# zz9tf/multimodal-fusion

Measured on AMD Instinct MI355X. Metric: similarity-pairs/sec (NxN cosine+top-k), higher is better.
Workload: dtype f16 MFMA scan + f32 exact re-rank; 1 GPU; N=262144 d=512 single-modality cosine + top-5, self excluded, f32 features, unit-norm Gaussian rows; rows_per_rank=262144, parallelism=single GPU, driver=single, scan_kernel=scan_b16x<f16> (v_mfma_f32_16x16x32_f16), col_splits=1, scan_grid=2048, fallback_rows=0, overflow_rows=0, query_order=False, near_duplicate_rows_estimate=0

## Files before the change

multimodal-fusion_amd/csrc/mmf_api.hip:

```cpp
#include <stdarg.h>
#include <string.h>

#include <algorithm>
#include <map>
#include <mutex>
#include <optional>
#include <utility>
#include <vector>

#include "mmf_host.h"

namespace mmf {

static thread_local char g_err[512] = "";

void set_error(const char* fmt, ...) {
  va_list ap;
  va_start(ap, fmt);
  vsnprintf(g_err, sizeof(g_err), fmt, ap);
  va_end(ap);
}

struct WsEntry { char* base = nullptr; size_t cap = 0; WsKept kept; };
static std::mutex g_ws_mu;
// ... 213 lines not shown

static void fill_stats(mmf_simtopk_stats* st, int precision, int splits, int grid, float prep_ms, float scan_ms, float rerank_ms,
                       float fallback_ms, int64_t fallback_rows, int64_t overflow_rows, int64_t short_rows,
                       const std::vector<uint32_t>& h_tot, int64_t near_rows = -1) {
  if (!st) return;
  st->precision_used = precision; st->col_splits = splits; st->scan_grid = grid;
  st->prep_ms = prep_ms; st->scan_ms = scan_ms; st->rerank_ms = rerank_ms; st->fallback_ms = fallback_ms;
  st->fallback_rows = fallback_rows; st->overflow_rows = overflow_rows; st->short_rows = short_rows;
  for (uint32_t v : h_tot) st->candidates += v;
  st->near_rows = near_rows;
}

static constexpr int kSpillCap = 192;

static size_t b16_lists_bytes(int64_t n, int lists, int bcap) {
  const size_t e = (size_t)n * lists;
  return ws_bytes(e, 4) + ws_bytes(e * bcap, 4) + (lists > 2 ? ws_bytes(e * bcap, 4) + ws_bytes(n, 4) : 0) + 2 * ws_bytes(n, 4) +
         ws_bytes((size_t)n * kSpillCap, 4);
}
static CandLists carve_b16_lists(Workspace& ws, int64_t n, int lists, int bcap) {
  CandLists L{};
  L.lists = lists; L.cap = bcap; L.slot_ulp = scan_bf16_slot_ulp(bcap); L.spill_cap = kSpillCap;
  L.cnt = ws.take<uint32_t>((size_t)n * lists); L.ids = ws.take<uint32_t>((size_t)n * lists * bcap);
  if (lists > 2) { L.keys = ws.take<float>((size_t)n * lists * bcap); L.margin = ws.take<float>(n); }
  L.overflow = ws.take<uint32_t>(n); L.spill_cnt = ws.take<uint32_t>(n); L.spill_ids = ws.take<uint32_t>((size_t)n * kSpillCap);
  L.spill_stacks = (lists == 2 && !getenv("MMF_SPILL_COUNTER")) ? 1 : 0;
  return L;
}

struct FlagBlock {
  int32_t* fail_rows = nullptr; uint32_t *fail_count = nullptr, *cand_total = nullptr;
  uint32_t h_fail4[4] = {0, 0, 0, 0};
  std::vector<uint32_t> h_tot;
  static size_t bytes(int64_t n) { return ws_bytes(n, 4) + ws_bytes(4, 4) + ws_bytes(256, 4); }
  void carve(Workspace& ws, int64_t n) { fail_rows = ws.take<int32_t>(n); fail_count = ws.take<uint32_t>(4); cand_total = ws.take<uint32_t>(256); }
  int zero(hipStream_t s) const {
    MMF_HIP(hipMemsetAsync(fail_count, 0, 16, s)); MMF_HIP(hipMemsetAsync(cand_total, 0, 1024, s));
    return MMF_OK;
  }
  int read(bool totals, hipStream_t s) {
    MMF_HIP(hipMemcpyAsync(h_fail4, fail_count, 16, hipMemcpyDeviceToHost, s));
    h_tot.assign(totals ? 256 : 0, 0);
    if (totals) MMF_HIP(hipMemcpyAsync(h_tot.data(), cand_total, 1024, hipMemcpyDeviceToHost, s));
    MMF_HIP(hipStreamSynchronize(s));
    return MMF_OK;
  }
};

static void symmetric_live_mode(bool* live, bool* forward) {
  const char* e = getenv("MMF_SYMMETRIC_LIVE");
  const int v = e ? atoi(e) : 1;
  *live = (v == 1 || v == 2);
  *forward = (v == 0 || v == 2);
}
static constexpr int64_t kSymMinRows = 131072;
static bool symmetric_scan_wanted(int64_t n, int dp, int bcap, int metric, int forced_splits, bool same_ids, int* G) {
  if (!same_ids || dp != 512 || bcap != scan_bf16_cap(1, 512) || forced_splits != 0) return false;
  if (metric != MMF_DOT && metric != MMF_COSINE) return false;
  const int64_t nb = (n + 255) / 256;
  if (nb * 256 * 1024 >= (int64_t(1) << 32)) return false;
  const char* e = getenv("MMF_SYMMETRIC");
  const int mode = e ? atoi(e) : -1;
  if (mode == 0 || (mode < 0 && n < kSymMinRows)) return false;
  int g = sym_default_group(nb);
  if (const char* ge = getenv("MMF_SYMMETRIC_G")) { const int v = atoi(ge); if (v >= 1 && v <= 65536) g = v; }
  *G = g;
  return true;
}


struct ExactLists {
  CandLists L{};
  int32_t* fail_rows = nullptr; uint32_t* fail_count = nullptr;
  float* floor_key = nullptr; uint32_t* floor_id = nullptr;
  int64_t rows = 0;
  static size_t bytes(int64_t rows, size_t list_words, int cap, bool floors) {
    return ws_bytes(list_words, 4) + ws_bytes(list_words * cap, 4) + (floors ? 4 : 2) * ws_bytes(rows, 4) + ws_bytes(4, 4);
  }
  void carve(Workspace& ws, int64_t rows_, size_t list_words, int cap, bool floors) {
    rows = rows_;
    L.cnt = ws.take<uint32_t>(list_words); L.ids = ws.take<uint32_t>(list_words * cap); L.overflow = ws.take<uint32_t>(rows);
    fail_rows = ws.take<int32_t>(rows); fail_count = ws.take<uint32_t>(4);
    if (floors) { floor_key = ws.take<float>(rows); floor_id = ws.take<uint32_t>(rows); }
  }
  int zero(hipStream_t s) const {
    MMF_HIP(hipMemsetAsync(fail_count, 0, 16, s)); MMF_HIP(hipMemsetAsync(L.overflow, 0, (size_t)rows * 4, s));
    return MMF_OK;
  }
};

struct ExactGroup {
  int64_t row0, rows;
  bool gathered;
  int64_t col0, cols;
  int k;
};

struct ExactPass {
  static constexpr int64_t kBatch = 4096;
  const Request& r;
  const float *rx, *cy;
  bool same = false;
  int forced_splits = 0;
  const int32_t* row_ids = nullptr;
  int64_t n_ids = 0;
  uint32_t* cand_total = nullptr;
// ... 192 lines not shown
  void carve(Workspace& ws) {
    L = carve_b16_lists(ws, n, lists_alloc, bcap);
    if (sym_try) {
      sym_cnt = ws.take<uint32_t>(n); sym_ids = ws.take<uint32_t>((size_t)n * kSymCap); sym_keys = ws.take<float>((size_t)n * kSymCap);
      sym.carve(ws, n_pad_q(), sym_grid());
      sym_kept = ws.kept; sym_keep = ws.keep;
    }
    flags.carve(ws, n);
    XL.carve(ws, FB, (size_t)FB * 2 * fb_splits, cap, false);
    scan_scratch = ws.take<char>(scan_scratch_bytes());
    seed = ws.take<int32_t>(2 * n_seed);
    row_keys = ws.take<float>((size_t)rows_exact_cap * m);
    order_scratch = ws.take<char>(select_order_bytes(n));
    if (order_try) {
      qo_scratch = ws.take<char>(query_order_bytes(n));
      qo_Z = ws.take<uint16_t>((size_t)n_pad_q() * dp);
      qo_zn = ws.take<float>(n_pad_q()); qo_rn = ws.take<float>(n_pad_q()); qo_un = ws.take<float>(n_pad_q());
    }
  }
  int run(const Request& r, const FastOperands& fo_in, void* select_wait_event) {
    const hipStream_t s = r.call.s;
    const bool profile = r.profile;
    FastOperands fo = fo_in;
    query_order_forget();
    EventTimer t_order;
    int64_t near_rows = -1;
    if (order_try) {
      MMF_TRY(t_order.start(profile, s));
      MMF_TRY(launch_query_order_probe(fo.ZQ, fo.q_zn, n, fo.dp, fo.f16, qo_scratch, &near_rows, s));
      if (order_mode == MMF_QUERY_ORDER_ON || near_rows >= 8 * (int64_t)query_order_pivots()) {
        MMF_TRY(launch_query_order_apply(fo.ZQ, fo.q_zn, fo.q_rn, fo.q_un, n, n_pad_q(), fo.dp, fo.f16, qo_scratch, qo_Z, qo_zn, qo_rn, qo_un, &fo.perm, s));
        fo.ZQ = qo_Z; fo.q_zn = qo_zn; fo.q_rn = qo_rn; fo.q_un = qo_un;
      }
      MMF_TRY(t_order.stop(s));
    }
    const bool symmetric = sym_try && !fo.perm && fo.n_panels == 0;
    const CandLists L = view(symmetric);
    MMF_HIP(hipMemsetAsync(L.overflow, 0, (size_t)n * 4, s));
    MMF_TRY(flags.zero(s));
    EventTimer t_scan, t_sel, t_fb;
    EventTimer t_panel[16];
    int grid = 0;
    MMF_HIP(hipMemsetAsync(seed, 0x80, (size_t)n_seed * 8, s));
    MMF_HIP(hipMemsetAsync(L.spill_cnt, 0, (size_t)n * 4, s));
    MMF_TRY(t_scan.start(profile, s));
    ScanB16Panel pn;
    pn.seed = seed; pn.seed_stride = n_seed;
    pn.share = (splits > 1 || fo.n_panels > 1) ? 1 : 0;
    if (symmetric) {
      bool live, forward;
      symmetric_live_mode(&live, &forward);
      const WsKept tables{sym.sched, (n + 255) / 256, sym_G, forward ? 1 : 0};
      MMF_TRY(launch_scan_b16_sym(fo.ZC, fo.c_cb, fo.q_zn, fo.q_rn, fo.q_un, fo.max_c, n, r.d, fo.f16, r.metric, kk, sym_G, live, forward,
                                  !(sym_kept == tables), L, scan_scratch, sym, pn, s, &grid));
      if (sym_keep) *sym_keep = tables;
    } else if (fo.n_panels == 0) {
      MMF_TRY(launch_scan_b16(fo.ZQ, fo.ZC, fo.c_cb, fo.q_zn, fo.q_rn, fo.q_un, fo.max_c, n, m, fo.m_pad_tiles, fo.dp, r.d, fo.f16,
                              r.metric, kk, splits, L, scan_scratch, pn, s, &grid));
    } else {
      int list_base = 0;
      for (int p = 0; p < fo.n_panels; ++p) {
        const mmf_panel& P = fo.panels[p];
        if (P.ready_event) MMF_HIP(hipStreamWaitEvent(s, static_cast<hipEvent_t>(P.ready_event), 0));
        MMF_TRY(t_panel[p].start(profile, s));
        pn.list_base = list_base;
        list_base += 2 * panel_splits[p];
        pn.seg_len = (uint32_t)P.seg_len; pn.seg_stride = (uint32_t)P.seg_stride; pn.id_off = (uint32_t)P.id_base;
        MMF_TRY(launch_scan_b16(fo.ZQ, P.Z, P.cb, fo.q_zn, fo.q_rn, fo.q_un, fo.max_c, n, P.m, P.m_pad, fo.dp, r.d, fo.f16,
                                r.metric, kk, panel_splits[p], L, scan_scratch, pn, s, &grid));
        MMF_TRY(t_panel[p].stop(s));
      }
    }
    MMF_TRY(launch_scan_b16_audit(pn, L.overflow, n, s));
    if (const char* e = getenv("MMF_DEBUG_FLAG_ROWS")) {
      const int64_t f = atoll(e);
      if (f > 0) MMF_HIP(hipMemsetAsync(L.overflow, 1, (size_t)(f < n ? f : n) * 4, s));
    }
    MMF_TRY(t_scan.stop(s));
    if (symmetric && getenv("MMF_SYMMETRIC_DEBUG")) {
      MMF_HIP(hipStreamSynchronize(s));
      std::vector<uint32_t> hc((size_t)n), hl((size_t)sym_grid() * 8);
      uint32_t none = 0;
      MMF_HIP(hipMemcpy(hc.data(), sym_cnt, hc.size() * 4, hipMemcpyDeviceToHost));
      MMF_HIP(hipMemcpy(hl.data(), sym.log_cnt, hl.size() * 4, hipMemcpyDeviceToHost));
      MMF_HIP(hipMemcpy(&none, sym.none_cnt, 4, hipMemcpyDeviceToHost));
      unsigned long long tot = 0; uint32_t mx = 0, lmx = 0;
      for (uint32_t v : hc) { tot += v; if (v > mx) mx = v; }
      for (uint32_t v : hl) if (v > lmx) lmx = v;
      bool live, forward;
      symmetric_live_mode(&live, &forward);
      fprintf(stderr, "[mmf symmetric] G %d grid %lld %s %s: rows without a threshold %u, received entries %llu (%.1f per row, largest %u of %d), fullest wave log %u of %d\n",
              sym_G, (long long)sym_grid(), live ? "live" : "frozen", forward ? "ahead" : "back", none, tot, (double)tot / (double)n, mx,
              kSymCap, lmx, kSymLogPerWave);
    }
    if (select_wait_event) MMF_HIP(hipStreamWaitEvent(s, static_cast<hipEvent_t>(select_wait_event), 0));

    SelectProblem q = r.select();
    q.rx = fo.rx; q.cy = fo.cy; q.perm = fo.perm;
    q.fail_rows = flags.fail_rows; q.fail_count = flags.fail_count; q.cand_total = r.stats ? flags.cand_total : nullptr;
    q.two_pass = true;
    q.order_scratch = getenv("MMF_SELECT_UNORDERED") ? nullptr : order_scratch;
    MMF_TRY(t_sel.start(profile, s));
    MMF_TRY(launch_select(q, L, s));
    MMF_TRY(t_sel.stop(s));

    MMF_TRY(flags.read(r.stats != nullptr, s));
    const uint32_t* h_fail4 = flags.h_fail4;
    const uint32_t h_fail = h_fail4[0];
    if (h_fail > 0 && getenv("MMF_DEBUG_PRINT_FLAGGED")) {
      const uint32_t nshow = h_fail < 8 ? h_fail : 8;
      int32_t rows[8];
      MMF_HIP(hipMemcpy(rows, flags.fail_rows, nshow * sizeof(int32_t), hipMemcpyDeviceToHost));
      for (uint32_t i = 0; i < nshow; ++i) {
        int32_t enc[2] = {0, 0};
        MMF_HIP(hipMemcpy(&enc[0], seed + rows[i], 4, hipMemcpyDeviceToHost));
        MMF_HIP(hipMemcpy(&enc[1], seed + n_seed + rows[i], 4, hipMemcpyDeviceToHost));
        auto dec = [](int32_t o) { int32_t b = o >= 0 ? o : (o ^ 0x7fffffff); float f; memcpy(&f, &b, 4); return f; };
        fprintf(stderr, "[mmf flagged] row %d: best threshold %.9g (enc %d)  best dropped key %.9g (enc %d)  overflow %u short %u\n",
                rows[i], dec(enc[0]), enc[0], dec(enc[1]), enc[1], h_fail4[1], h_fail4[2]);
      }
    }

    MMF_TRY(t_fb.start(profile && h_fail > 0, s));
    if (h_fail > 0 && (int64_t)h_fail <= kRowsExactMax) {
      for (int64_t off = 0; off < (int64_t)h_fail; off += rows_exact_cap) {
        SelectProblem fq = q;
        fq.perm = nullptr;
        fq.row_ids = flags.fail_rows + off;
        fq.n_rows = ((int64_t)h_fail - off < rows_exact_cap) ? ((int64_t)h_fail - off) : rows_exact_cap;
        MMF_TRY(launch_rows_exact(fq, row_keys, s));
      }
    } else if (h_fail > 0) {
      ExactPass ex(r, fo.rx, fo.cy);
      ex.row_ids = flags.fail_rows; ex.n_ids = h_fail; ex.forced_splits = fb_splits;
      ex.add(ExactGroup{0, (int64_t)h_fail, true, 0, m, r.k});
      Workspace aux;
      MMF_TRY(r.call.workspace(ex.image_bytes(), &aux, 1));
      MMF_TRY(XL.zero(s));
      MMF_TRY(ex.run(aux, XL));
    }
    MMF_TRY(t_fb.stop(s));
    fill_stats(r.stats, r.precision, symmetric ? 1 : splits, grid, 0.f, t_scan.ms(), t_sel.ms(), t_fb.ms(), h_fail, h_fail4[1], h_fail4[2], flags.h_tot,
               near_rows);
    if (r.stats) {
      if (profile && fo.n_panels > 0) {
        float launches = 0.f;
// ... 1086 lines not shown
```

multimodal-fusion_amd/csrc/mmf_host.h:

```cpp
#pragma once
#include <hip/hip_runtime.h>
#include <functional>
#include <optional>
#include <stdint.h>
#include <stdio.h>

#include <string>
#include <vector>

#include "../../include/mmf_hg.h"

namespace mmf {

void set_error(const char* fmt, ...);

#define MMF_HIP(call)                                                                      \
  do {                                                                                     \
    hipError_t _e = (call);                                                                \
    if (_e != hipSuccess) {                                                                \
      mmf::set_error("%s failed: %s (%s:%d)", #call, hipGetErrorString(_e), __FILE__, __LINE__); \
      return MMF_E_HIP;                                                                    \
    }                                                                                      \
  } while (0)

// ... 162 lines not shown
  int col_splits;
  const float* floor_key = nullptr;
  const uint32_t* floor_id = nullptr;
};

int scan_f32_cap(int kk);
int launch_scan_f32(const ScanProblem& p, const CandLists& L, hipStream_t s, int* grid_out);

struct SelectProblem {
  const void* X; int64_t n; const void* Y; int64_t m; int64_t d; int dtype; int metric; float lambda;
  int k; int exclude_self; int64_t row_offset; int64_t col_offset;
  const float* rx; const float* cy;
  const int32_t* row_ids; int64_t n_rows;
  int64_t* out_idx; float* out_val;
  int32_t* fail_rows; uint32_t* fail_count;
  uint32_t* cand_total;
  bool two_pass = false;
  int out_stride = 0, out_off = 0;
  float* floor_key_out = nullptr;
  uint32_t* floor_id_out = nullptr;
  void* order_scratch = nullptr;
  const int32_t* perm = nullptr;
};
size_t select_order_bytes(int64_t n);
size_t query_order_bytes(int64_t n);
int query_order_pivots();
int query_order_last(int32_t* out_host, int64_t n);
void query_order_forget();
int launch_query_order_probe(const uint16_t* ZQ, const float* q_zn, int64_t n, int dp, bool f16, void* scratch, int64_t* near, hipStream_t s);
int launch_query_order_apply(const uint16_t* ZQ, const float* q_zn, const float* q_rn, const float* q_un, int64_t n, int64_t n_pad,
                             int dp, bool f16, void* scratch, uint16_t* Zo, float* zno, float* rno, float* uno, const int32_t** perm,
                             hipStream_t s);
int launch_select(const SelectProblem& p, const CandLists& L, hipStream_t s);
int launch_rows_exact(const SelectProblem& p, float* keys, hipStream_t s);
int launch_topk_merge(const int64_t* ia, const float* va, const int64_t* ib, const float* vb,
                      int64_t n, int k, int64_t* io, float* vo, hipStream_t s);
int launch_edge_cosine_impl(const void* X, int64_t d, int dtype, const float* nrm, const int64_t* ei, int64_t E,
                            float* out, hipStream_t s);

int scan_bf16_supported(int64_t d, int kk, int dtype);
int scan_bf16_cap(int kk, int dp);
int scan_bf16_dp(int64_t d);
int launch_prep_half(const void* X, int64_t n, int64_t d, int dtype, int metric, const float* scal,
                     const uint32_t* max_n, void* Z,
                     int64_t n_pad, int dp, int z_f16, float* zn, float* rn, float* un, float* cb, uint32_t* maxima,
                     hipStream_t s);
int launch_scan_b16(const void* ZQ, const void* ZC, const float* cb, const float* q_zn, const float* q_rn,
                    const float* q_un, const uint32_t* maxima, int64_t n_rows, int64_t m, int64_t m_pad, int dp,
                    int64_t d, bool f16, int metric, int kk, int col_splits, const CandLists& L, void* scratch,
                    const ScanB16Panel& pn, hipStream_t s, int* grid_out);
int launch_scan_b16_audit(const ScanB16Panel& pn, uint32_t* overflow, int64_t n_rows, hipStream_t s);
size_t scan_b16_sym_scratch_bytes(int64_t n_rows, int G);
int launch_scan_b16_sym(const void* ZC, const float* cb, const float* zn, const float* rn, const float* un, const uint32_t* maxima,
                        int64_t n, int64_t d, bool f16, int metric, int kk, int G, bool live, bool forward, bool tables,
                        const CandLists& L, void* scratch, const SymBuffers& sb, const ScanB16Panel& pn, hipStream_t s, int* grid_out);
size_t scan_b16_scratch_bytes(int64_t n_rows, int col_splits, int dp, int cap);
int scan_bf16_slot_ulp(int cap);
int scan_b16_queries_per_block(int dp);
int launch_prep_half_gather(const void* X, int64_t n, int64_t d, int dtype, int metric, const float* scal,
                            const uint32_t* max_n, const int32_t* gather, void* Z, int64_t n_pos, int64_t n_pad, int dp,
                            int z_f16, float* zn, float* rn, float* un, float* cb, uint32_t* maxima, hipStream_t s);
size_t scan_b16_seg_scratch_bytes(int64_t grid, int dp, int cap);
int launch_scan_b16_seg(const void* ZQ, const void* ZC, const float* cb, const float* q_zn, const float* q_rn,
                        const float* q_un, const uint32_t* maxima, const int32_t* sched, int64_t grid, int64_t n_rows,
                        int64_t m, int dp, int64_t d, bool f16, int metric, int kk, const CandLists& L, void* scratch,
                        const ScanB16Panel& pn, hipStream_t s);

bool sim_dense_needs_images(int64_t d, int metric);
int launch_sim_dense(const void* X, int64_t n, const void* Y, int64_t m, int64_t d, int dtype,
                     int metric, float lambda, const float* rx, const float* cy, const float* Xp, const float* Yp,
                     float* out, hipStream_t s);
int launch_sim_dense_combined(const float* Fp, const float* P, int64_t n, int64_t d, int64_t dp,
                              float lambda_h, float lambda_g, const float* nf, int64_t row0, int64_t rows, float* out,
                              hipStream_t s);
std::vector<int64_t> sim_dense_combined_seg_table(const int64_t* ptr, int64_t S);
int launch_sim_dense_combined_seg(const float* Fp, const float* P, int64_t d, int64_t dp, float lambda_h, float lambda_g,
                                  const float* nf, const int64_t* sched, int64_t grid, float* out, hipStream_t s);

using MedianConsume = std::function<int(const float* data, int64_t cols, int64_t row0, int64_t rows)>;
using MedianSweep = std::function<int(const MedianConsume&)>;
using MedianSampler = std::function<int(float* sample, int s)>;
size_t median_scratch_bytes(unsigned long long count);
int64_t median_no_diagonal_row();
struct SweepCarry {
  void* lanes;
  int64_t grid;
  int64_t row0;
};
int lower_median_of(unsigned long long count, const MedianSampler& sampler, const MedianSweep& sweep, float* out, void* scratch,
                    hipStream_t s, void* stat_part = nullptr, const float* stat_pivot = nullptr, int64_t* stat_nparts = nullptr,
                    SweepCarry* carry = nullptr);
bool median_one_sweep(unsigned long long count);
size_t stat_lanes_bytes(int64_t grid);
int launch_stat_lanes_init(void* lanes, int64_t grid, hipStream_t s);
int launch_stat_lanes_finish(void* lanes, int64_t grid, void* part , hipStream_t s);
int64_t stats_partial_grid(int64_t count);
int launch_stats_partial_carry(const float* v, int64_t count, int64_t group0, const float* pivot, void* lanes, int64_t grid, hipStream_t s);
int launch_sample_gather(const float* data, int64_t n_sq, unsigned long long count, float* sample, int s_count, hipStream_t s);
int launch_sample_pairs(const void* A, const void* B, int64_t nb, int64_t d, int dtype, float lambda, const float* P, int dp,
                        float lambda_g, int offdiag, unsigned long long count, float* sample, int s_count, hipStream_t s);
int launch_offdiag_lower_median(const float* K, int64_t n, float* out, void* scratch ,
                                hipStream_t s);
int launch_median_accumulate(const float* K, int64_t n, int64_t row0, int64_t rows, void* state, int pass, hipStream_t s);
int launch_median_next(void* state, int pass, float* out, hipStream_t s);
int launch_median_begin_count(void* state, unsigned long long count, hipStream_t s);
int launch_lower_median(const float* v, int64_t count, float* out, void* scratch, hipStream_t s);
int launch_stats_finish(const void* part, int64_t nparts, const float* pivot, int64_t count, double* out, hipStream_t s);
// ... 71 lines not shown
```

multimodal-fusion_amd/csrc/mmf_scan_bf16.hip:

```cpp
#include <stdlib.h>

#include <type_traits>

#include "mmf_dev.h"
#include "mmf_host.h"

namespace mmf {

constexpr int B_CT = 32;
#ifndef MMF_B_CAP
#define MMF_B_CAP 15
#endif
constexpr int B_CAP = MMF_B_CAP;
constexpr int B_CAP_BIG = 16;
constexpr int B_CAP_WIDE = 32;

typedef __bf16 bf16x8_t __attribute__((ext_vector_type(8)));
typedef _Float16 f16x8_t __attribute__((ext_vector_type(8)));
typedef uint32_t u32x4 __attribute__((ext_vector_type(4)));

struct PrepArgs {
  const void* X; int64_t n; int64_t d; int dtype; int metric;
  const float* scal;
  const uint32_t* max_n;
// ... 111 lines not shown
  const void* ZC;
  const float* cb;
  const float* q_zn; const float* q_rn; const float* q_un;
  const uint32_t* maxima;
  int64_t n_rows;
  int64_t m;
  int64_t tiles_total;
  int64_t tiles_per_split;
  int64_t row_blocks;
  int col_splits;
  int conc_splits;
  int64_t blocks_per_round;
  int lists_total;
  int list_base;
  uint32_t seg_len, seg_stride, id_off;
  int32_t* seed;
  int32_t* lost;
  int share;
  int kk;
  int metric;
  int d;
  int debug;
  unsigned long long* dbg;
  uint32_t* lids;
  uint32_t* cand_cnt; uint32_t* cand_ids; uint32_t* overflow;
  float* cand_keys;
  float* margin_out;
  uint32_t* spill_cnt; uint32_t* spill_ids; int spill_cap;
  int spill_stacks;
  const int32_t* sched;
  float* sym_thr;
  int sym_live;
  uint32_t* sym_log;
  uint32_t* sym_log_cnt;
  int sym_log_cap;
};

enum { SEG_QPOS = 0, SEG_ROW0 = 1, SEG_NQ = 2, SEG_T0 = 3, SEG_T1 = 4, SEG_IDOFF = 5, SEG_ENTRY = 8 };
enum { SYM_RB = 0, SYM_B1 = 1, SYM_N1 = 2, SYM_B2 = 3, SYM_N2 = 4 };

__device__ __forceinline__ int32_t seed_enc(float f) {
  const int32_t b = __float_as_int(f);
  return b >= 0 ? b : (b ^ 0x7fffffff);
}
constexpr int32_t kSeedNone = (int32_t)0x80808080;

__device__ __forceinline__ void glds4(const void* gptr, const void* lptr) {
  __builtin_amdgcn_global_load_lds((const __attribute__((address_space(1))) void*)(gptr), (__attribute__((address_space(3))) void*)(lptr), 4, 0, 0);
}

#ifndef MMF_SYM_ABLATE
#define MMF_SYM_ABLATE 0
#endif
template <int KS, bool F16, bool DBG, int NW, int TPB, int CAP, bool SPLITK = false, bool SEG = false, int SYM = 0>
__global__ __launch_bounds__(64 * NW, (NW == 8) ? 2 : 1) void scan_b16x_kernel(ScanB16Args a) {
  static_assert(!SPLITK || (TPB == 1 && NW == 8 && (KS % 8) == 0), "split-k pairs");
  static_assert(SYM == 0 || (!SPLITK && !SEG && !DBG && TPB == 2), "symmetric schedule: the d = 512 kernel only");
  constexpr int NQW = SPLITK ? NW / 2 : NW;
  constexpr int NTL = 64 * NQW;
  constexpr int QT = 32 * NQW;
  constexpr int STAGES = 2 * TPB;
  constexpr int ROWB = KS * 32;
  constexpr int TILEB = B_CT * ROWB;
  constexpr int PIECES = TILEB / 1024;
  constexpr int PPW = (PIECES + NW - 1) / NW;
  static_assert(PIECES % NW == 0, "piece distribution");
  extern __shared__ __attribute__((aligned(1024))) char smem[];
  char* tiles = smem;
  float* cbs = reinterpret_cast<float*>(smem + STAGES * TILEB);
  float* lkeys = cbs + STAGES * 64;
  uint32_t* lids = a.lids + (size_t)blockIdx.x * (SlotList<CAP, NTL>::SLOTS * NTL);
  f32x4* xch = reinterpret_cast<f32x4*>(lkeys + CAP * NTL);
  volatile int* ack = reinterpret_cast<volatile int*>(xch + NQW * 4 * 64);

  const int tid = threadIdx.x;
  const int lane = tid & 63;
  const int wave = __builtin_amdgcn_readfirstlane(tid >> 6);
  const int khalf = SPLITK ? wave / NQW : 0;
  const int qw = SPLITK ? wave % NQW : wave;
  const bool owner = khalf == 0;
  const int half = lane >> 5;
  const int g = lane >> 4;
  const int c16 = lane & 15;
  const int ownb = g & 1;
  const int c = c16 + 16 * ownb;

  int64_t rb;
  int split;
  int64_t t_begin, t_end, row0 = 0;
  int nq = 0;
  uint32_t id_off = a.id_off;
  int sym_n1 = 0, sym_skip = 0;
  if constexpr (SYM != 0) {
    const int32_t* e = a.sched + (size_t)blockIdx.x * SEG_ENTRY;
    if (e[SYM_RB] < 0) return;
    rb = e[SYM_RB]; split = 0;
    t_begin = e[SYM_B1]; t_end = t_begin + e[SYM_N1] + e[SYM_N2];
    sym_n1 = e[SYM_N1]; sym_skip = e[SYM_B2] - (e[SYM_B1] + e[SYM_N1]);
  } else if constexpr (SEG) {
    const int32_t* e = a.sched + (size_t)blockIdx.x * SEG_ENTRY;
    rb = e[SEG_QPOS] / QT; row0 = e[SEG_ROW0]; nq = e[SEG_NQ];
    t_begin = e[SEG_T0]; t_end = e[SEG_T1]; id_off = (uint32_t)e[SEG_IDOFF];
    split = 0;
  } else {
    const int CS = a.conc_splits;
    const int64_t round = blockIdx.x / a.blocks_per_round;
// ... 67 lines not shown
  u32x4 qf[KS2][2];
  {
    const char* qbase = reinterpret_cast<const char*>(a.ZQ) + (q0 + 32 * qw + c16) * (int64_t)ROWB + g * 16 + kbyte;
#pragma unroll
    for (int s = 0; s < KS2; ++s) {
      qf[s][0] = *reinterpret_cast<const u32x4*>(qbase + s * 64);
      qf[s][1] = *reinterpret_cast<const u32x4*>(qbase + 16 * (int64_t)ROWB + s * 64);
    }
#pragma unroll
    for (int s = 0; s < KS2; ++s) { asm volatile("" : "+v"(qf[s][0])); asm volatile("" : "+v"(qf[s][1])); }
  }

  int lo[4];
#pragma unroll
  for (int j = 0; j < 4; ++j) lo[j] = c16 * ROWB + ((((4 * j + g) ^ c16) & 15) << 4);

  uint32_t src_off[PPW];
#pragma unroll
  for (int i = 0; i < PPW; ++i) {
    const int p = wave + NW * i;
    const int off = p * 1024 + lane * 16;
    const int r = off / ROWB;
    const int chunk = (off % ROWB) >> 4;
    const int src_chunk = (chunk & ~15) | ((chunk ^ r) & 15);
    src_off[i] = (uint32_t)(r * ROWB + src_chunk * 16);
  }
  const char* zc0 = reinterpret_cast<const char*>(a.ZC) + (SYM != 0 ? 0 : t_begin * (int64_t)TILEB);
  const char* cb0 = reinterpret_cast<const char*>(a.cb + (SYM != 0 ? 0 : t_begin * B_CT));
  const char* zt0 = SYM != 0 ? zc0 + t_begin * (int64_t)TILEB : zc0;
  const char* ct0 = SYM != 0 ? cb0 + t_begin * B_CT * 4 : cb0;
  const __amdgpu_buffer_rsrc_t zrsrc = __builtin_amdgcn_make_buffer_rsrc(const_cast<char*>(zc0), 0, -1, 0x00020000);
  auto issue_piece = [&](const char* tsrc, int stage, int i) {
    if (DBG && (a.debug & 2)) return;
    if (DBG && (a.debug & 32)) tsrc = zc0;
    __builtin_amdgcn_raw_ptr_buffer_load_lds(zrsrc, (__attribute__((address_space(3))) void*)(tiles + stage * TILEB + (wave + NW * i) * 1024),
                                             16, (int)src_off[i], (int)(uint32_t)(tsrc - zc0), 0, 0);
  };
  const __amdgpu_buffer_rsrc_t brsrc = __builtin_amdgcn_make_buffer_rsrc(const_cast<char*>(cb0), 0, -1, 0x00020000);
  auto issue_bias = [&](const char* bsrc, int stage) {
    const uint32_t l = __builtin_amdgcn_mbcnt_hi(~0u, __builtin_amdgcn_mbcnt_lo(~0u, 0u));
    if (l < 32)
      __builtin_amdgcn_raw_ptr_buffer_load_lds(brsrc, (__attribute__((address_space(3))) void*)(cbs + stage * 64), 4, (int)(l * 4u),
                                               (int)(uint32_t)(bsrc - cb0), 0, 0);
  };
  auto sym_thr_stage = [&](int stage) -> float* { return lkeys + CAP * NTL + stage * 32; };
  auto issue_thr = [&](const char* bsrc, int stage) {
    const __amdgpu_buffer_rsrc_t trsrc = __builtin_amdgcn_make_buffer_rsrc(a.sym_thr, 0, -1, 0x00020000);
    const uint32_t l = __builtin_amdgcn_mbcnt_hi(~0u, __builtin_amdgcn_mbcnt_lo(~0u, 0u));
    if (l < 32)
      __builtin_amdgcn_raw_ptr_buffer_load_lds(trsrc, (__attribute__((address_space(3))) void*)sym_thr_stage(stage), 4, (int)(l * 4u),
                                               (int)(uint32_t)(bsrc - cb0), 0, 16);
  };

  if (SPLITK && tid < NQW) ack[tid] = -1;
  const int Ti = (int)T;
  if (Ti > 0) {
#pragma unroll
    for (int u = 0; u < TPB; ++u) {
      const bool real = u < Ti;
#pragma unroll
      for (int i = 0; i < PPW; ++i) issue_piece(real ? zt0 + u * (int64_t)TILEB : zc0, u, i);
      if (wave == (u & (NW - 1))) issue_bias(real ? ct0 + u * B_CT * 4 : cb0, u);
      if constexpr (SYM == 2) { if (wave == ((u + 4) & (NW - 1))) issue_thr(real ? ct0 + u * B_CT * 4 : cb0, u); }
    }
  }
  constexpr int GRP = KS2 / PPW;
  static_assert(KS2 % PPW == 0 && GRP >= 1, "DMA piece placement");
  const char* tsrc = zt0 + TPB * (int64_t)TILEB;
  const char* bsrc = ct0 + TPB * B_CT * 4;
  const uint32_t id_base = (uint32_t)(t_begin * B_CT);

  struct Acc { f32x4 t[2][2]; };
  auto tile_body = [&](const char* tb, const float* cbt, const char* src, int s2) -> Acc {
    Acc acc;
#pragma unroll
    for (int cb = 0; cb < 2; ++cb) {
      f32x4 b4 = *reinterpret_cast<const f32x4*>(cbt + 16 * cb + 4 * g);
      if (SPLITK && !owner) b4 = f32x4{0.f, 0.f, 0.f, 0.f};
      acc.t[cb][0] = b4; acc.t[cb][1] = b4;
    }
    constexpr int PD = 2;
    u32x4 af[PD][2];
#pragma unroll
    for (int s = 0; s < PD; ++s) {
      af[s][0] = *reinterpret_cast<const u32x4*>(tb + lo[s & 3] + (s >> 2) * 256);
      af[s][1] = *reinterpret_cast<const u32x4*>(tb + lo[s & 3] + (s >> 2) * 256 + 16 * ROWB);
    }
    __builtin_amdgcn_sched_group_barrier(0x100, 2 * PD, 0);
#pragma unroll
    for (int s = 0; s < KS2; ++s) {
      const u32x4 a0 = af[s % PD][0], a1 = af[s % PD][1];
      if (s + PD < KS2) {
        af[s % PD][0] = *reinterpret_cast<const u32x4*>(tb + lo[(s + PD) & 3] + ((s + PD) >> 2) * 256);
        af[s % PD][1] = *reinterpret_cast<const u32x4*>(tb + lo[(s + PD) & 3] + ((s + PD) >> 2) * 256 + 16 * ROWB);
      }
      if constexpr (F16) {
        acc.t[0][0] = __builtin_amdgcn_mfma_f32_16x16x32_f16(__builtin_bit_cast(f16x8_t, a0), __builtin_bit_cast(f16x8_t, qf[s][0]), acc.t[0][0], 0, 0, 0);
        acc.t[0][1] = __builtin_amdgcn_mfma_f32_16x16x32_f16(__builtin_bit_cast(f16x8_t, a0), __builtin_bit_cast(f16x8_t, qf[s][1]), acc.t[0][1], 0, 0, 0);
        acc.t[1][0] = __builtin_amdgcn_mfma_f32_16x16x32_f16(__builtin_bit_cast(f16x8_t, a1), __builtin_bit_cast(f16x8_t, qf[s][0]), acc.t[1][0], 0, 0, 0);
        acc.t[1][1] = __builtin_amdgcn_mfma_f32_16x16x32_f16(__builtin_bit_cast(f16x8_t, a1), __builtin_bit_cast(f16x8_t, qf[s][1]), acc.t[1][1], 0, 0, 0);
      } else {
        acc.t[0][0] = __builtin_amdgcn_mfma_f32_16x16x32_bf16(__builtin_bit_cast(bf16x8_t, a0), __builtin_bit_cast(bf16x8_t, qf[s][0]), acc.t[0][0], 0, 0, 0);
        acc.t[0][1] = __builtin_amdgcn_mfma_f32_16x16x32_bf16(__builtin_bit_cast(bf16x8_t, a0), __builtin_bit_cast(bf16x8_t, qf[s][1]), acc.t[0][1], 0, 0, 0);
        acc.t[1][0] = __builtin_amdgcn_mfma_f32_16x16x32_bf16(__builtin_bit_cast(bf16x8_t, a1), __builtin_bit_cast(bf16x8_t, qf[s][0]), acc.t[1][0], 0, 0, 0);
        acc.t[1][1] = __builtin_amdgcn_mfma_f32_16x16x32_bf16(__builtin_bit_cast(bf16x8_t, a1), __builtin_bit_cast(bf16x8_t, qf[s][1]), acc.t[1][1], 0, 0, 0);
      }
      if ((s % GRP) == GRP - 1) issue_piece(src, s2, s / GRP);
      if (s + PD < KS2) __builtin_amdgcn_sched_group_barrier(0x100, 2, 0);
      __builtin_amdgcn_sched_group_barrier(0x008, 4, 0);
    }
    return acc;
  };
  auto max_qb = [&](const Acc& x, int qb) -> float {
    const f32x4& p = x.t[0][qb];
    const f32x4& q = x.t[1][qb];
    return fmaxf(fmaxf(fmaxf(p[0], p[1]), fmaxf(p[2], p[3])), fmaxf(fmaxf(q[0], q[1]), fmaxf(q[2], q[3])));
  };
  float thr_q0, thr_q1;
  auto refresh_thr = [&]() {
    const float mine = list.thr;
    const float theirs = __shfl_xor(mine, 16);
    thr_q0 = ownb ? theirs : mine;
    thr_q1 = ownb ? mine : theirs;
  };
  refresh_thr();

  auto filter = [&](const Acc& acc, int tt, float m0, float m1) {
    if (__builtin_expect(!(DBG && (a.debug & 1)) && __any((m0 >= thr_q0) || (m1 >= thr_q1)), 0)) {
      uint32_t id0 = id_base + (uint32_t)tt * B_CT;
      if constexpr (SYM != 0) id0 += (tt >= sym_n1) ? (uint32_t)(sym_skip * B_CT) : 0u;
      f32x16 v;
#pragma unroll
      for (int cb = 0; cb < 2; ++cb) {
#pragma unroll
        for (int j = 0; j < 4; ++j) {
          const float mine = ownb ? acc.t[cb][1][j] : acc.t[cb][0][j];
          const float give = ownb ? acc.t[cb][0][j] : acc.t[cb][1][j];
          v[4 * cb + j] = mine;
          v[8 + 4 * cb + j] = __shfl_xor(give, 16);
        }
      }
      const int g4 = 4 * g;
      auto rowof = [g4](int r) -> uint32_t { return (uint32_t)((g4 ^ ((r & 8) >> 1)) + (r & 3) + 16 * ((r >> 2) & 1)); };
      const bool cold = (!seeded && tt < 32) || __any(list.thr == -kFltMax);
      if (DBG && (a.debug & 8)) {
        const bool willc = __any(list.cnt >= CAP - 1);
        int nh = 0;
#pragma unroll
        for (int r = 0; r < 16; ++r) nh += (v[r] >= list.thr) ? 1 : 0;
        const int lanes_hit = __popcll(__ballot(nh > 0));
#pragma unroll
        for (int o = 32; o > 0; o >>= 1) nh += __shfl_xor(nh, o);
        if (lane == 0) {
          atomicAdd(a.dbg + 0, 1ull);
          atomicAdd(a.dbg + 1, cold ? 1ull : 0ull);
          atomicAdd(a.dbg + 2, (unsigned long long)nh);
          atomicAdd(a.dbg + 3, (!cold && willc) ? 1ull : 0ull);
          atomicAdd(a.dbg + 4, (unsigned long long)lanes_hit);
        }
      }
      unsigned long long ts0 = 0;
      if (DBG && (a.debug & 16)) ts0 = __builtin_amdgcn_s_memtime();
      list.offer_tile(v, id0, rowof, a.kk, margin);
      if (DBG && (a.debug & 16) && lane == 0) {
        const unsigned long long dt = __builtin_amdgcn_s_memtime() - ts0;
        atomicAdd(a.dbg + (cold ? 4 : 5), dt);
        atomicAdd(a.dbg + (cold ? 6 : 7), 1ull);
      }
      refresh_thr();
// ... 53 lines not shown
        }
        sym_wcnt += (uint32_t)__popcll(busy);
        busy = __ballot(m != 0u);
      }
    }
  };

  unsigned long long tw = 0, tf = 0, tc = 0, tv = 0, t0s = 0, t1s = 0, t2s = 0, t3s = 0, tvs = 0;
  const bool stamps = DBG && (a.debug & 16) != 0;
  Acc acc_prev;
  float m0_prev = kNegInf, m1_prev = kNegInf;
#pragma unroll
  for (int cb = 0; cb < 2; ++cb) {
#pragma unroll
    for (int j = 0; j < 4; ++j) { acc_prev.t[cb][0][j] = kNegInf; acc_prev.t[cb][1][j] = kNegInf; }
  }
  const int nIter = (Ti + TPB - 1) / TPB;
  for (int j = 0; j < nIter; ++j) {
    if (stamps) tvs = __builtin_amdgcn_s_memtime();
    __builtin_amdgcn_s_waitcnt(0x0F70);
    if (stamps) t0s = __builtin_amdgcn_s_memtime();
    asm volatile("" ::: "memory");
    if (!(DBG && (a.debug & 4)))
    __builtin_amdgcn_s_barrier();
    asm volatile("" ::: "memory");
    if (stamps) t1s = __builtin_amdgcn_s_memtime();

    if constexpr (SPLITK) {
      if (owner) {
        if (j > 0) {
#pragma unroll
          for (int i = 0; i < 4; ++i) {
            const f32x4 p = xch[(qw * 4 + i) * 64 + lane];
            acc_prev.t[i >> 1][i & 1] += p;
          }
          m0_prev = max_qb(acc_prev, 0);
          m1_prev = max_qb(acc_prev, 1);
        }
        asm volatile("" ::: "memory");
        if (lane == 0) ack[qw] = j;
      }
    }
    if (owner) filter(acc_prev, j * TPB - 1, m0_prev, m1_prev);
    if (stamps) t2s = __builtin_amdgcn_s_memtime();

    const int sg = (j & 1) * TPB, ng = TPB - sg;
#pragma unroll
    for (int u = 0; u < TPB; ++u) {
      const int t = j * TPB + u;
      const bool more = (t + TPB < Ti);
      const char* src = more ? tsrc + u * (int64_t)TILEB : zc0;
      Acc acc;
      acc = tile_body(tiles + (sg + u) * TILEB + kbyte, cbs + (sg + u) * 64, src, ng + u);
      if (wave == ((t + TPB) & (NW - 1))) issue_bias(more ? bsrc + u * B_CT * 4 : cb0, ng + u);
      if constexpr (SYM == 2 && MMF_SYM_ABLATE != 2) {
        if (wave == ((t + TPB + 4) & (NW - 1))) issue_thr(more ? bsrc + u * B_CT * 4 : cb0, ng + u);
        if (t < Ti) sym_offer(acc, t, sym_thr_stage(sg + u));
      }
      if (u < TPB - 1) {
        if (TPB == 2 || __builtin_expect(t < Ti, 1))
        filter(acc, t, max_qb(acc, 0), max_qb(acc, 1));
      } else {
        if (__builtin_expect(t >= Ti, 0)) {
#pragma unroll
          for (int cb = 0; cb < 2; ++cb) {
#pragma unroll
            for (int jj = 0; jj < 4; ++jj) { acc.t[cb][0][jj] = kNegInf; acc.t[cb][1][jj] = kNegInf; }
          }
        }
        acc_prev = acc;
        if constexpr (!SPLITK) {
          m0_prev = max_qb(acc, 0);
          m1_prev = max_qb(acc, 1);
        } else if (!owner) {
          while (ack[qw] < j) __builtin_amdgcn_s_sleep(1);
          asm volatile("" ::: "memory");
#pragma unroll
          for (int i = 0; i < 4; ++i) xch[(qw * 4 + i) * 64 + lane] = acc.t[i >> 1][i & 1];
          __builtin_amdgcn_s_waitcnt(0xC07F);
        }
      }
    }
    tsrc += TPB * (int64_t)TILEB;
    bsrc += TPB * B_CT * 4;
    if constexpr (SYM != 0) {
      if ((j + 2) * TPB == sym_n1) { tsrc += sym_skip * (int64_t)TILEB; bsrc += sym_skip * (B_CT * 4); }
    }
    if (stamps) {
      asm volatile("" :: "v"(acc_prev.t[0][0][0]));
      t3s = __builtin_amdgcn_s_memtime();
      tw += t1s - t0s; tf += t2s - t1s; tc += t3s - t2s; tv += t0s - tvs;
    }
  }
  if (stamps && lane == 0) {
    atomicAdd(a.dbg + 0, tw); atomicAdd(a.dbg + 1, tf); atomicAdd(a.dbg + 2, tc); atomicAdd(a.dbg + 3, (unsigned long long)Ti);
    atomicAdd(a.dbg + 8, tv);
  }
  if constexpr (SPLITK) {
    __builtin_amdgcn_s_waitcnt(0x0F70);
    __builtin_amdgcn_s_barrier();
    if (owner && Ti > 0) {
#pragma unroll
      for (int i = 0; i < 4; ++i) acc_prev.t[i >> 1][i & 1] += xch[(qw * 4 + i) * 64 + lane];
    }
  }
  if (Ti > 0 && owner) filter(acc_prev, nIter * TPB - 1, max_qb(acc_prev, 0), max_qb(acc_prev, 1));
  __builtin_amdgcn_s_waitcnt(0x0F70);

  list.compact(a.kk, margin);
// ... 256 lines not shown
int sym_default_group(int64_t nb) {
  int64_t g = (nb + 31) / 32;
  return (int)(g < 32 ? 32 : g);
}
static int64_t sym_super_blocks(int64_t nb, int G) { const int64_t ns = nb / G; return ns < 1 ? 1 : ns; }
int64_t sym_schedule_grid(int64_t nb, int G) {
  const int64_t ns = sym_super_blocks(nb, G);
  return ((ns + 7) / 8 + (nb > ns * G ? 1 : 0)) * 8 * G;
}
void sym_schedule_table(int64_t nb, int G, int launch, int32_t* out, bool forward) {
  const int64_t ns = sym_super_blocks(nb, G), grid = sym_schedule_grid(nb, G), tiles = nb * 8;
  const int64_t per = 8 * (int64_t)G, stretches = (ns + 7) / 8;
  auto first_tile = [&](int64_t sb) { return sb * G * 8; };
  auto end_tile = [&](int64_t sb) { return sb == ns - 1 ? tiles : (sb + 1) * G * 8; };
  for (int64_t b = 0; b < grid; ++b) {
    int32_t* e = out + b * SEG_ENTRY;
    for (int i = 0; i < SEG_ENTRY; ++i) e[i] = 0;
    e[SYM_RB] = -1;
    int64_t sb = (b / per) * 8 + (b % 8), rbi = sb * G + (b % per) / 8;
    if (b / per >= stretches) {
      if (b % 8 != (ns - 1) % 8) continue;
      sb = ns - 1; rbi = ns * G + (b % per) / 8;
    } else if (sb >= ns) continue;
    if (rbi >= nb) continue;
    int64_t b1 = 0, n1 = 0, b2 = 0, n2 = 0;
    if (launch == 0) {
      b1 = first_tile(sb); n1 = end_tile(sb) - b1;
      if (ns >= 2 && (ns % 2) == 0) { const int64_t o = (sb + ns / 2) % ns; b2 = first_tile(o); n2 = end_tile(o) - b2; }
    } else {
      const int64_t h = (ns - 1) / 2;
      if (h == 0) continue;
      int64_t lo = forward ? sb + 1 : sb - h, hi = lo + h - 1;
      if (lo >= ns) { lo -= ns; hi -= ns; }
      if (lo < 0) { lo += ns; hi += ns; }
      if (hi < ns) { b1 = first_tile(lo); n1 = end_tile(hi) - b1; }
      else { b1 = first_tile(lo); n1 = end_tile(ns - 1) - b1; b2 = 0; n2 = end_tile(hi - ns); }
    }
    if (n2 == 0) b2 = b1 + n1;
    e[SYM_RB] = (int32_t)rbi; e[SYM_B1] = (int32_t)b1; e[SYM_N1] = (int32_t)n1; e[SYM_B2] = (int32_t)b2; e[SYM_N2] = (int32_t)n2;
  }
}

__global__ void sym_thr_kernel(const int32_t* seed, float* thr, int64_t n, int64_t n_pad, uint32_t* none_cnt) {
  const int64_t i = (int64_t)blockIdx.x * blockDim.x + threadIdx.x;
  if (i >= n_pad) return;
  if (i >= n) { thr[i] = __builtin_huge_valf(); return; }
  const int32_t o = seed[i];
  if (o > kSeedNone) { thr[i] = __int_as_float(o >= 0 ? o : (o ^ 0x7fffffff)); return; }
  thr[i] = -kFltMax;
  atomicAdd(none_cnt, 1u);
}

__global__ __launch_bounds__(256) void sym_scatter_kernel(const uint32_t* log, const uint32_t* log_cnt, int log_cap, uint32_t* sym_cnt,
                                                          uint32_t* sym_ids, float* sym_keys, int cap, int32_t* lost) {
  const uint32_t c = log_cnt[blockIdx.x];
  const u32x4* lg = reinterpret_cast<const u32x4*>(log) + (size_t)blockIdx.x * log_cap;
  for (uint32_t e = threadIdx.x; e < c; e += 256) {
    const u32x4 v = lg[e];
    const uint32_t slot = atomicAdd(sym_cnt + v[0], 1u);
    if (slot < (uint32_t)cap) {
      sym_ids[(size_t)v[0] * cap + slot] = v[1];
      sym_keys[(size_t)v[0] * cap + slot] = __uint_as_float(v[2]);
    } else {
      atomicMax(lost + v[0], 0x7fffffff);
    }
  }
}

size_t scan_b16_sym_scratch_bytes(int64_t n_rows, int G) {
  const int64_t nb = (n_rows + 255) / 256;
  return (size_t)sym_schedule_grid(nb, G) * 16 * 512 * 4 + 256;
}

int launch_scan_b16_sym(const void* ZC, const float* cb, const float* zn, const float* rn, const float* un, const uint32_t* maxima,
                        int64_t n, int64_t d, bool f16, int metric, int kk, int G, bool live, bool forward, bool tables,
                        const CandLists& L, void* scratch, const SymBuffers& sb, const ScanB16Panel& pn, hipStream_t s, int* grid_out) {
  const int64_t nb = (n + 255) / 256, n_pad = nb * 256, grid = sym_schedule_grid(nb, G);
  if (L.lists != 4 || L.cap != B_CAP || !L.keys || !L.margin || !L.sym_cnt || !pn.seed) { set_error("scan_b16_sym: lists missing"); return MMF_E_INTERNAL; }
  if (n_pad * 1024 >= (int64_t(1) << 32)) { set_error("scan_b16_sym: operand image beyond the 32-bit tile offsets"); return MMF_E_INTERNAL; }
  if (tables) {
    std::vector<int32_t> tab((size_t)grid * 2 * SEG_ENTRY);
    sym_schedule_table(nb, G, 0, tab.data(), forward);
    sym_schedule_table(nb, G, 1, tab.data() + (size_t)grid * SEG_ENTRY, forward);
    MMF_TRY(upload_table(s, sb.sched, tab.data(), tab.size() * 4));
  }
  MMF_HIP(hipMemsetAsync(L.sym_cnt, 0, (size_t)n * 4, s));
  MMF_HIP(hipMemsetAsync(L.cnt, 0, (size_t)n * L.lists * 4, s));
  MMF_HIP(hipMemsetAsync(sb.log_cnt, 0, (size_t)grid * 8 * 4, s));
  MMF_HIP(hipMemsetAsync(sb.none_cnt, 0, 16, s));
  ScanB16Args a{};
  a.ZQ = ZC; a.ZC = ZC; a.cb = cb; a.q_zn = zn; a.q_rn = rn; a.q_un = un; a.maxima = maxima;
  a.n_rows = n; a.m = n; a.tiles_total = n_pad / B_CT; a.tiles_per_split = 0;
  a.row_blocks = nb; a.col_splits = 1; a.conc_splits = 1; a.blocks_per_round = 0;
  a.kk = kk; a.metric = metric; a.d = (int)d;
  a.lists_total = L.lists; a.list_base = 0;
  a.seed = pn.seed; a.lost = pn.seed + pn.seed_stride; a.share = 0;
  a.cand_cnt = L.cnt; a.cand_ids = L.ids; a.overflow = L.overflow; a.cand_keys = L.keys; a.margin_out = L.margin;
  a.spill_cnt = L.spill_cnt; a.spill_ids = L.spill_ids; a.spill_cap = L.spill_cap; a.spill_stacks = 0;
  a.lids = reinterpret_cast<uint32_t*>(scratch);
  a.sched = sb.sched;
  a.sym_thr = sb.thr; a.sym_live = live ? 1 : 0; a.sym_log = sb.log; a.sym_log_cnt = sb.log_cnt; a.sym_log_cap = kSymLogPerWave;
  auto go = [&](auto kern, size_t lds) -> int {
    MMF_HIP(hipFuncSetAttribute(reinterpret_cast<const void*>(kern), hipFuncAttributeMaxDynamicSharedMemorySize, (int)lds));
    hipLaunchKernelGGL(kern, dim3((unsigned)grid), dim3(512), lds, s, a);
    MMF_LAUNCH_CHECK();
    return MMF_OK;
  };
  const size_t lds_a = scan_b16_lds(32, 8, 2, B_CAP, false), lds_b = scan_b16_lds(32, 8, 2, B_CAP, false, true);
  if (f16) MMF_TRY(go(scan_b16x_kernel<32, true, false, 8, 2, B_CAP, false, false, 1>, lds_a));
  else MMF_TRY(go(scan_b16x_kernel<32, false, false, 8, 2, B_CAP, false, false, 1>, lds_a));
  hipLaunchKernelGGL(sym_thr_kernel, dim3((unsigned)((n_pad + 255) / 256)), dim3(256), 0, s, pn.seed, sb.thr, n, n_pad, sb.none_cnt);
  MMF_LAUNCH_CHECK();
  a.sched = sb.sched + (size_t)grid * SEG_ENTRY; a.list_base = 2; a.share = 1;
  if (f16) MMF_TRY(go(scan_b16x_kernel<32, true, false, 8, 2, B_CAP, false, false, 2>, lds_b));
  else MMF_TRY(go(scan_b16x_kernel<32, false, false, 8, 2, B_CAP, false, false, 2>, lds_b));
  hipLaunchKernelGGL(sym_scatter_kernel, dim3((unsigned)(grid * 8)), dim3(256), 0, s, sb.log, sb.log_cnt, kSymLogPerWave, L.sym_cnt,
                     L.sym_ids, L.sym_keys, L.sym_cap, pn.seed + pn.seed_stride);
  MMF_LAUNCH_CHECK();
  if (grid_out) *grid_out = (int)(2 * grid);
  return MMF_OK;
}

}
```

Measured before the change: 2005 billion pairs/s.

## Drop bias loads in symmetric scan, batch threshold loads, prune scatter entries

In the symmetric scan kernels, accumulators now start at zero instead of loading a per-candidate bias tile, and padding columns are masked to -inf explicitly. Threshold tiles are fetched as one paired DMA per tile group rather than one per tile. The scatter kernel drops logged entries that already fall below the row's seed threshold before taking an atomic slot, which can be turned off with an environment variable. This reduces memory traffic and atomics, but the symmetric path now rejects metrics that need a bias, and the masking must match the removed bias behavior.

```diff
diff --git a/multimodal-fusion_amd/csrc/mmf_api.hip b/multimodal-fusion_amd/csrc/mmf_api.hip
--- a/multimodal-fusion_amd/csrc/mmf_api.hip
+++ b/multimodal-fusion_amd/csrc/mmf_api.hip
@@ -289,6 +289,10 @@
   const int v = e ? atoi(e) : 1;
   *live = (v == 1 || v == 2);
   *forward = (v == 0 || v == 2);
+}
+static bool symmetric_prune_mode() {
+  const char* e = getenv("MMF_SYMMETRIC_PRUNE");
+  return !e || atoi(e) != 0;
 }
 static constexpr int64_t kSymMinRows = 131072;
 static bool symmetric_scan_wanted(int64_t n, int dp, int bcap, int metric, int forced_splits, bool same_ids, int* G) {
@@ -587,7 +591,7 @@
       symmetric_live_mode(&live, &forward);
       const WsKept tables{sym.sched, (n + 255) / 256, sym_G, forward ? 1 : 0};
       MMF_TRY(launch_scan_b16_sym(fo.ZC, fo.c_cb, fo.q_zn, fo.q_rn, fo.q_un, fo.max_c, n, r.d, fo.f16, r.metric, kk, sym_G, live, forward,
-                                  !(sym_kept == tables), L, scan_scratch, sym, pn, s, &grid));
+                                  symmetric_prune_mode(), !(sym_kept == tables), L, scan_scratch, sym, pn, s, &grid));
       if (sym_keep) *sym_keep = tables;
     } else if (fo.n_panels == 0) {
       MMF_TRY(launch_scan_b16(fo.ZQ, fo.ZC, fo.c_cb, fo.q_zn, fo.q_rn, fo.q_un, fo.max_c, n, m, fo.m_pad_tiles, fo.dp, r.d, fo.f16,
@@ -619,14 +623,14 @@
       MMF_HIP(hipMemcpy(hc.data(), sym_cnt, hc.size() * 4, hipMemcpyDeviceToHost));
       MMF_HIP(hipMemcpy(hl.data(), sym.log_cnt, hl.size() * 4, hipMemcpyDeviceToHost));
       MMF_HIP(hipMemcpy(&none, sym.none_cnt, 4, hipMemcpyDeviceToHost));
-      unsigned long long tot = 0; uint32_t mx = 0, lmx = 0;
+      unsigned long long tot = 0, logged = 0; uint32_t mx = 0, lmx = 0;
       for (uint32_t v : hc) { tot += v; if (v > mx) mx = v; }
-      for (uint32_t v : hl) if (v > lmx) lmx = v;
+      for (uint32_t v : hl) { logged += v; if (v > lmx) lmx = v; }
       bool live, forward;
       symmetric_live_mode(&live, &forward);
-      fprintf(stderr, "[mmf symmetric] G %d grid %lld %s %s: rows without a threshold %u, received entries %llu (%.1f per row, largest %u of %d), fullest wave log %u of %d\n",
+      fprintf(stderr, "[mmf symmetric] G %d grid %lld %s %s: rows without a threshold %u, received entries %llu (%.1f per row, largest %u of %d), fullest wave log %u of %d, logged entries %llu (%.1f per row, filing %s)\n",
               sym_G, (long long)sym_grid(), live ? "live" : "frozen", forward ? "ahead" : "back", none, tot, (double)tot / (double)n, mx,
-              kSymCap, lmx, kSymLogPerWave);
+              kSymCap, lmx, kSymLogPerWave, logged, (double)logged / (double)n, symmetric_prune_mode() ? "pruned" : "complete");
     }
     if (select_wait_event) MMF_HIP(hipStreamWaitEvent(s, static_cast<hipEvent_t>(select_wait_event), 0));
 
diff --git a/multimodal-fusion_amd/csrc/mmf_host.h b/multimodal-fusion_amd/csrc/mmf_host.h
--- a/multimodal-fusion_amd/csrc/mmf_host.h
+++ b/multimodal-fusion_amd/csrc/mmf_host.h
@@ -238,7 +238,7 @@
 int launch_scan_b16_audit(const ScanB16Panel& pn, uint32_t* overflow, int64_t n_rows, hipStream_t s);
 size_t scan_b16_sym_scratch_bytes(int64_t n_rows, int G);
 int launch_scan_b16_sym(const void* ZC, const float* cb, const float* zn, const float* rn, const float* un, const uint32_t* maxima,
-                        int64_t n, int64_t d, bool f16, int metric, int kk, int G, bool live, bool forward, bool tables,
+                        int64_t n, int64_t d, bool f16, int metric, int kk, int G, bool live, bool forward, bool prune, bool tables,
                         const CandLists& L, void* scratch, const SymBuffers& sb, const ScanB16Panel& pn, hipStream_t s, int* grid_out);
 size_t scan_b16_scratch_bytes(int64_t n_rows, int col_splits, int dp, int cap);
 int scan_bf16_slot_ulp(int cap);
diff --git a/multimodal-fusion_amd/csrc/mmf_scan_bf16.hip b/multimodal-fusion_amd/csrc/mmf_scan_bf16.hip
--- a/multimodal-fusion_amd/csrc/mmf_scan_bf16.hip
+++ b/multimodal-fusion_amd/csrc/mmf_scan_bf16.hip
@@ -187,6 +187,9 @@
 #ifndef MMF_SYM_ABLATE
 #define MMF_SYM_ABLATE 0
 #endif
+#ifndef MMF_SYM_EARLY_THR
+#define MMF_SYM_EARLY_THR 1
+#endif
 template <int KS, bool F16, bool DBG, int NW, int TPB, int CAP, bool SPLITK = false, bool SEG = false, int SYM = 0>
 __global__ __launch_bounds__(64 * NW, (NW == 8) ? 2 : 1) void scan_b16x_kernel(ScanB16Args a) {
   static_assert(!SPLITK || (TPB == 1 && NW == 8 && (KS % 8) == 0), "split-k pairs");
@@ -360,6 +363,13 @@
                                                (int)(uint32_t)(bsrc - cb0), 0, 16);
   };
 
+  auto issue_thr_pair = [&](const char* bsrc, int stage) {
+    const __amdgpu_buffer_rsrc_t trsrc = __builtin_amdgcn_make_buffer_rsrc(a.sym_thr, 0, -1, 0x00020000);
+    const uint32_t l = __builtin_amdgcn_mbcnt_hi(~0u, __builtin_amdgcn_mbcnt_lo(~0u, 0u));
+    __builtin_amdgcn_raw_ptr_buffer_load_lds(trsrc, (__attribute__((address_space(3))) void*)sym_thr_stage(stage), 4, (int)(l * 4u),
+                                             (int)(uint32_t)(bsrc - cb0), 0, 16);
+  };
+
   if (SPLITK && tid < NQW) ack[tid] = -1;
   const int Ti = (int)T;
   if (Ti > 0) {
@@ -368,9 +378,10 @@
       const bool real = u < Ti;
 #pragma unroll
       for (int i = 0; i < PPW; ++i) issue_piece(real ? zt0 + u * (int64_t)TILEB : zc0, u, i);
-      if (wave == (u & (NW - 1))) issue_bias(real ? ct0 + u * B_CT * 4 : cb0, u);
-      if constexpr (SYM == 2) { if (wave == ((u + 4) & (NW - 1))) issue_thr(real ? ct0 + u * B_CT * 4 : cb0, u); }
-    }
+      if constexpr (SYM == 0) { if (wave == (u & (NW - 1))) issue_bias(real ? ct0 + u * B_CT * 4 : cb0, u); }
+      if constexpr (SYM == 2 && !MMF_SYM_EARLY_THR) { if (wave == ((u + 4) & (NW - 1))) issue_thr(real ? ct0 + u * B_CT * 4 : cb0, u); }
+    }
+    if constexpr (SYM == 2 && MMF_SYM_EARLY_THR) { if (wave == 4) issue_thr_pair(Ti >= TPB ? ct0 : cb0, 0); }
   }
   constexpr int GRP = KS2 / PPW;
   static_assert(KS2 % PPW == 0 && GRP >= 1, "DMA piece placement");
@@ -381,11 +392,16 @@
   struct Acc { f32x4 t[2][2]; };
   auto tile_body = [&](const char* tb, const float* cbt, const char* src, int s2) -> Acc {
     Acc acc;
+    if constexpr (SYM != 0) {
+#pragma unroll
+      for (int cb = 0; cb < 2; ++cb) { acc.t[cb][0] = f32x4{0.f, 0.f, 0.f, 0.f}; acc.t[cb][1] = f32x4{0.f, 0.f, 0.f, 0.f}; }
+    } else {
 #pragma unroll
     for (int cb = 0; cb < 2; ++cb) {
       f32x4 b4 = *reinterpret_cast<const f32x4*>(cbt + 16 * cb + 4 * g);
       if (SPLITK && !owner) b4 = f32x4{0.f, 0.f, 0.f, 0.f};
       acc.t[cb][0] = b4; acc.t[cb][1] = b4;
+    }
     }
     constexpr int PD = 2;
     u32x4 af[PD][2];
@@ -423,6 +439,18 @@
     const f32x4& p = x.t[0][qb];
     const f32x4& q = x.t[1][qb];
     return fmaxf(fmaxf(fmaxf(p[0], p[1]), fmaxf(p[2], p[3])), fmaxf(fmaxf(q[0], q[1]), fmaxf(q[2], q[3])));
+  };
+  auto mask_padding = [&](Acc& x, int tt) {
+    const int64_t r0 = (int64_t)id_base + (int64_t)tt * B_CT + ((tt >= sym_n1) ? (int64_t)sym_skip * B_CT : 0);
+    if (__builtin_expect(r0 + B_CT > a.m, 0)) {
+#pragma unroll
+      for (int cb = 0; cb < 2; ++cb) {
+#pragma unroll
+        for (int jj = 0; jj < 4; ++jj) {
+          if (r0 + 16 * cb + 4 * g + jj >= a.m) { x.t[cb][0][jj] = kNegInf; x.t[cb][1][jj] = kNegInf; }
+        }
+      }
+    }
   };
   float thr_q0, thr_q1;
   auto refresh_thr = [&]() {
@@ -582,9 +610,11 @@
       const char* src = more ? tsrc + u * (int64_t)TILEB : zc0;
       Acc acc;
       acc = tile_body(tiles + (sg + u) * TILEB + kbyte, cbs + (sg + u) * 64, src, ng + u);
-      if (wave == ((t + TPB) & (NW - 1))) issue_bias(more ? bsrc + u * B_CT * 4 : cb0, ng + u);
+      if constexpr (SYM == 0) { if (wave == ((t + TPB) & (NW - 1))) issue_bias(more ? bsrc + u * B_CT * 4 : cb0, ng + u); }
+      else mask_padding(acc, t);
       if constexpr (SYM == 2 && MMF_SYM_ABLATE != 2) {
-        if (wave == ((t + TPB + 4) & (NW - 1))) issue_thr(more ? bsrc + u * B_CT * 4 : cb0, ng + u);
+        if constexpr (MMF_SYM_EARLY_THR) { if (u == 0 && wave == (j & (NW - 1))) issue_thr_pair(more ? bsrc : cb0, ng); }
+        else if (wave == ((t + TPB + 4) & (NW - 1))) issue_thr(more ? bsrc + u * B_CT * 4 : cb0, ng + u);
         if (t < Ti) sym_offer(acc, t, sym_thr_stage(sg + u));
       }
       if (u < TPB - 1) {
@@ -947,11 +977,16 @@
 }
 
 __global__ __launch_bounds__(256) void sym_scatter_kernel(const uint32_t* log, const uint32_t* log_cnt, int log_cap, uint32_t* sym_cnt,
-                                                          uint32_t* sym_ids, float* sym_keys, int cap, int32_t* lost) {
+                                                          uint32_t* sym_ids, float* sym_keys, int cap, int32_t* lost,
+                                                          const int32_t* seed, int slot_ulp) {
   const uint32_t c = log_cnt[blockIdx.x];
   const u32x4* lg = reinterpret_cast<const u32x4*>(log) + (size_t)blockIdx.x * log_cap;
   for (uint32_t e = threadIdx.x; e < c; e += 256) {
     const u32x4 v = lg[e];
+    if (seed) {
+      const int32_t sd = seed[v[0]], b = (int32_t)v[2];
+      if (sd > kSeedNone && (b >= 0 ? b : (b ^ 0x7fffffff)) + slot_ulp < sd) continue;
+    }
     const uint32_t slot = atomicAdd(sym_cnt + v[0], 1u);
     if (slot < (uint32_t)cap) {
       sym_ids[(size_t)v[0] * cap + slot] = v[1];
@@ -968,9 +1003,13 @@
 }
 
 int launch_scan_b16_sym(const void* ZC, const float* cb, const float* zn, const float* rn, const float* un, const uint32_t* maxima,
-                        int64_t n, int64_t d, bool f16, int metric, int kk, int G, bool live, bool forward, bool tables,
+                        int64_t n, int64_t d, bool f16, int metric, int kk, int G, bool live, bool forward, bool prune, bool tables,
                         const CandLists& L, void* scratch, const SymBuffers& sb, const ScanB16Panel& pn, hipStream_t s, int* grid_out) {
   const int64_t nb = (n + 255) / 256, n_pad = nb * 256, grid = sym_schedule_grid(nb, G);
+  if (metric != MMF_DOT && metric != MMF_COSINE) {
+    set_error("scan_b16_sym: metric %d has a per-candidate bias, which the symmetric kernels do not apply", metric);
+    return MMF_E_INTERNAL;
+  }
   if (L.lists != 4 || L.cap != B_CAP || !L.keys || !L.margin || !L.sym_cnt || !pn.seed) { set_error("scan_b16_sym: lists missing"); return MMF_E_INTERNAL; }
   if (n_pad * 1024 >= (int64_t(1) << 32)) { set_error("scan_b16_sym: operand image beyond the 32-bit tile offsets"); return MMF_E_INTERNAL; }
   if (tables) {
@@ -1010,7 +1049,7 @@
   if (f16) MMF_TRY(go(scan_b16x_kernel<32, true, false, 8, 2, B_CAP, false, false, 2>, lds_b));
   else MMF_TRY(go(scan_b16x_kernel<32, false, false, 8, 2, B_CAP, false, false, 2>, lds_b));
   hipLaunchKernelGGL(sym_scatter_kernel, dim3((unsigned)(grid * 8)), dim3(256), 0, s, sb.log, sb.log_cnt, kSymLogPerWave, L.sym_cnt,
-                     L.sym_ids, L.sym_keys, L.sym_cap, pn.seed + pn.seed_stride);
+                     L.sym_ids, L.sym_keys, L.sym_cap, pn.seed + pn.seed_stride, prune ? pn.seed : nullptr, L.slot_ulp);
   MMF_LAUNCH_CHECK();
   if (grid_out) *grid_out = (int)(2 * grid);
   return MMF_OK;
```

Measured after the change: 2048 billion pairs/s, median of 6. 1.02x the previous value.
